# soon-yau/upgpt

Measured on AMD Instinct MI355X. Metric: 256x256 images/sec, 50-step DDIM, bs=8/GPU; UNet MFMA util %, higher is better.
Workload: dtype f16; 1 GPU; BASELINE configs[1]: bs=8/GPU, 256x256 px (latent 4x32x32), 50-step DDIM eta=0, text-only cond [B,87,768], UNet(bbox.yaml) + VAE decode, EMA weights, no CFG; batch_per_gpu=8, ddim_steps=50, batches_in_flight_per_gpu=4, lane_hw_queues=measured, parallelism=replica-dp1, one all-gather of images per batch

## Files before the change

### include/upk.h

```cpp
#ifndef UPK_H_
#define UPK_H_

#include <stddef.h>
#include <stdint.h>

#ifdef __cplusplus
extern "C" {
#endif

#define UPK_VERSION 100

#define UPK_OK 0
#define UPK_EINVAL (-1)
#define UPK_ESHAPE (-2)
#define UPK_EWORKSPACE (-3)
#define UPK_EHIP (-4)
#define UPK_ENODEV (-5)

typedef struct upk_ctx upk_ctx;
typedef void* upk_stream;

int upk_version(void);
int upk_create(upk_ctx** out, int device);
int upk_destroy(upk_ctx* ctx);
// ... 17 lines not shown
typedef struct upk_conv_desc {
  const void* x1;
  const void* x2;
  int32_t c1, c2;
  int32_t ld1, ld2;
  int32_t batch;
  int32_t in_h, in_w;
  int32_t ksize;
  int32_t stride;
  const void* w_packed;
  int32_t n_out;
  int32_t n_pad;
  const float* bias;
  const void* residual;
  int32_t ld_res;
  const float* rowvec;
  int32_t rv_batch_stride;
  int32_t rv_step_stride;
  const int32_t* step;
  void* y;
  int32_t ldy;
  void* vt;
  int32_t vt_from, vt_heads, vt_dhead, vt_ld, vt_tokens;
  int32_t flags;
  int32_t tune_cfg, tune_splitk;
  const float* ln_colsum;
  float ln_eps;
  int32_t ln_dim;
  float* gn_stats_ws;
  int32_t gn_groups;
  const void* x3;
  const void* x4;
  int32_t c3, c4;
  int32_t ld3, ld4;
  const float* gno_gamma;
  const float* gno_beta;
  void* gno_y;
  float gno_eps;
  int32_t gno_silu, gno_ld, gno_skip_y;
  float* ln_rows_out;
  const float* ln_rows_in;
  int32_t ln_rows_slots;
  const void* w_phase;
  int32_t gn_stats_cap;
  const void* pf_next;
  int64_t pf_bytes;
} upk_conv_desc;

int upk_conv2d_nhwc_f16(upk_ctx* ctx, const upk_conv_desc* d, upk_stream stream);

int upk_conv_gn_fused(upk_ctx* ctx, const upk_conv_desc* d, int* mode, int* nblk);
int upk_groupnorm_finalize_f32(upk_ctx* ctx, const float* partials, int nblk, int ld, int batch, int hw, int c,
                               int groups, float* ws, upk_stream stream);
int upk_conv_ln_rows(upk_ctx* ctx, const upk_conv_desc* d, int* slots);

typedef struct upk_mlp_desc {
  const void* x;
  int32_t ldx, m, c, inner;
  const void* w1;
  const float* b1;
  const float* u1;
  float ln_eps;
  int32_t ln_dim;
  const void* w2;
  const float* b2;
  int32_t n_out, n_pad;
  const void* residual;
  int32_t ld_res;
  void* y;
  int32_t ldy;
  float* gn_stats_ws;
  int32_t hw, rows_per_wg;
} upk_mlp_desc;
int upk_geglu_mlp_f16(upk_ctx* ctx, const upk_mlp_desc* d, upk_stream stream);
int upk_geglu_mlp_supported(upk_ctx* ctx, const upk_mlp_desc* d);

typedef struct upk_xblock_desc {
  const void* a1;
  int32_t lda, m, c, heads, d;
  const void* t0;
  int32_t ld_t0;
  const void* w_out1;
  const void* w_q;
  const void* w_out2;
  const float* vec;
  float ln_eps;
  int32_t ln_dim;
  const void* k_ctx;
  int32_t ldk, n_kv;
  const void* vt_ctx;
  int32_t vt_ld;
  float scale;
  void* y;
  int32_t ldy;
  int32_t hw, rows_per_wg;
} upk_xblock_desc;
int upk_cross_block_f16(upk_ctx* ctx, const upk_xblock_desc* d, upk_stream stream);
int upk_cross_block_supported(upk_ctx* ctx, const upk_xblock_desc* d);

typedef struct upk_hblock_desc {
  const void* x;
  int32_t ldx, m, c, heads, d;
  const void* w_in;
  const void* w_qkv;
  const float* vec;
  float ln_eps;
// ... 194 lines not shown
```

### upgpt_amd/_lib.py

```python
import contextlib
import ctypes as C
import os
import threading

import torch
from ._check import require

_HERE = os.path.dirname(os.path.abspath(__file__))
LIB_PATH = os.environ.get("UPK_LIB") or os.path.join(_HERE, "libupk.so")

SYMBOLS = [
    "upk_version", "upk_create", "upk_destroy", "upk_last_error", "upk_set_workspace", "upk_num_cus",
    "upk_pack_weight_f16", "upk_packed_weight_bytes", "upk_conv2d_nhwc_f16", "upk_gemm_f16",
    "upk_conv_autotune", "upk_conv_override", "upk_conv_num_configs", "upk_conv_config_name", "upk_conv_gn_fused",
    "upk_conv_ln_rows",
    "upk_geglu_mlp_f16", "upk_geglu_mlp_supported", "upk_cross_block_f16", "upk_cross_block_supported", "upk_head_block_f16", "upk_head_block_supported",
    "upk_attention_f16", "upk_groupnorm_nhwc_f16", "upk_groupnorm_stats_nhwc_f16", "upk_groupnorm_chunks", "upk_groupnorm_apply_nhwc_f16", "upk_groupnorm_finalize_f32", "upk_groupnorm_ws_bytes",
    "upk_layernorm_f16", "upk_timestep_embed_f16",
    "upk_nchw_f32_to_nhwc_f16", "upk_nhwc_f16_to_nchw_f32", "upk_f32_to_f16", "upk_ddim_step_f32",
    "upk_ddim_step_cfg_f32", "upk_ddim_step_edit_f32", "upk_plms_step_f32", "upk_ddpm_step_f32", "upk_attention_causal_f16", "upk_attention_qproj_f16", "upk_embed_tokens_f16",
    "upk_patchify_nchw_f32_f16", "upk_vit_assemble_f16", "upk_gather_rows_f16",
    "upk_image_finish_u8", "upk_resize_bilinear_u8", "upk_segm_boxes_u8", "upk_style_crops_u8",
    "upk_cond_bbox_u8", "upk_cond_gather_u8", "upk_cond_smpl_u8", "upk_clip_normalize_u8", "upk_ssim_ws_bytes", "upk_ssim_u8",
    "upk_lpips_input_f16", "upk_relu_pool_nhwc_f16", "upk_lpips_ws_bytes", "upk_lpips_layer_f16",
    "upk_conv2d_rect_f16", "upk_pool3_nhwc_f16", "upk_fid_input_f16", "upk_avgpool_global_f32",
    "upk_advance_step", "upk_step_autoadvance", "upk_kernel_launches", "upk_graph_begin", "upk_graph_end", "upk_graph_launch", "upk_graph_destroy",
    "upk_prof_enable", "upk_prof_collect",
    "upk_stream_create_cumask", "upk_stream_destroy", "upk_probe_placement", "upk_probe_clock",
]

F_SILU, F_GEGLU, F_OUT_F32, F_OUT_NCHW_F32, F_UPSAMPLE2X, F_PAD_ASYM = 0x1, 0x2, 0x4, 0x8, 0x10, 0x20
DDPM_X0, DDPM_CLIP = 0x1, 0x2
LAYOUT_NCHW, LAYOUT_NHWC = 0, 1
STYLE_FILL, STYLE_MASK = 0x1, 0x2
FINISH_SAMPLE, FINISH_INPUT, FINISH_DENORM = 0, 1, 2
F_QUICKGELU = 0x40
POOL_MAX, POOL_AVG = 0, 1
NUM_CLASSES = 5
CLASS_NAMES = ["igemm", "attention", "groupnorm", "layernorm", "other"]

E_NAMES = {0: "UPK_OK", -1: "UPK_EINVAL", -2: "UPK_ESHAPE", -3: "UPK_EWORKSPACE", -4: "UPK_EHIP", -5: "UPK_ENODEV"}


class UpkError(RuntimeError):
    def __init__(self, code, msg):
        super().__init__("%s: %s" % (E_NAMES.get(code, str(code)), msg))
        self.code = code


class ConvDesc(C.Structure):
    _fields_ = [
        ("x1", C.c_void_p), ("x2", C.c_void_p),
        ("c1", C.c_int32), ("c2", C.c_int32), ("ld1", C.c_int32), ("ld2", C.c_int32),
        ("batch", C.c_int32), ("in_h", C.c_int32), ("in_w", C.c_int32),
        ("ksize", C.c_int32), ("stride", C.c_int32),
        ("w_packed", C.c_void_p), ("n_out", C.c_int32), ("n_pad", C.c_int32),
        ("bias", C.c_void_p), ("residual", C.c_void_p), ("ld_res", C.c_int32),
        ("rowvec", C.c_void_p), ("rv_batch_stride", C.c_int32), ("rv_step_stride", C.c_int32),
        ("step", C.c_void_p), ("y", C.c_void_p), ("ldy", C.c_int32),
        ("vt", C.c_void_p), ("vt_from", C.c_int32), ("vt_heads", C.c_int32), ("vt_dhead", C.c_int32),
        ("vt_ld", C.c_int32), ("vt_tokens", C.c_int32), ("flags", C.c_int32),
        ("tune_cfg", C.c_int32), ("tune_splitk", C.c_int32),
        ("ln_colsum", C.c_void_p), ("ln_eps", C.c_float), ("ln_dim", C.c_int32),
        ("gn_stats_ws", C.c_void_p), ("gn_groups", C.c_int32),
        ("x3", C.c_void_p), ("x4", C.c_void_p),
        ("c3", C.c_int32), ("c4", C.c_int32), ("ld3", C.c_int32), ("ld4", C.c_int32),
        ("gno_gamma", C.c_void_p), ("gno_beta", C.c_void_p), ("gno_y", C.c_void_p), ("gno_eps", C.c_float),
        ("gno_silu", C.c_int32), ("gno_ld", C.c_int32), ("gno_skip_y", C.c_int32),
        ("ln_rows_out", C.c_void_p), ("ln_rows_in", C.c_void_p), ("ln_rows_slots", C.c_int32),
        ("w_phase", C.c_void_p), ("gn_stats_cap", C.c_int32),
# ... 42 lines not shown
    global _lib
    with _lib_lock:
        if _lib is not None and path is None:
            return _lib
        p = path or LIB_PATH
        if not os.path.exists(p):
            raise RuntimeError(
                "libupk.so not found at %s: build it with `python -m upgpt_amd.build` "
                "(hipcc --offload-arch=gfx950). There is no CPU fallback." % p)
        lib = C.CDLL(p)
        vp, i32, i64, f32 = C.c_void_p, C.c_int, C.c_longlong, C.c_float
        protos = {
            "upk_version": (C.c_int, []),
            "upk_create": (C.c_int, [C.POINTER(vp), i32]),
            "upk_destroy": (C.c_int, [vp]),
            "upk_last_error": (C.c_char_p, [vp]),
            "upk_set_workspace": (C.c_int, [vp, vp, C.c_size_t]),
            "upk_num_cus": (C.c_int, [vp]),
            "upk_pack_weight_f16": (C.c_int, [vp, vp, i32, i32, i32, i32, vp, i32, vp, i32, vp, vp]),
            "upk_packed_weight_bytes": (C.c_size_t, [i32, i32, i32, i32]),
            "upk_conv2d_nhwc_f16": (C.c_int, [vp, C.POINTER(ConvDesc), vp]),
            "upk_gemm_f16": (C.c_int, [vp, vp, i32, i32, i32, vp, i32, i32, vp, vp, i32, vp, i32, i32, vp]),
            "upk_conv_autotune": (C.c_int, [vp, C.POINTER(ConvDesc), vp, i32, C.POINTER(C.c_int), C.POINTER(C.c_int),
                                            C.POINTER(C.c_float), C.POINTER(C.c_float)]),
            "upk_conv_override": (C.c_int, [vp, i32, i32]),
            "upk_conv_num_configs": (C.c_int, []),
            "upk_conv_config_name": (C.c_char_p, [i32]),
            "upk_conv_ln_rows": (C.c_int, [vp, C.POINTER(ConvDesc), C.POINTER(C.c_int)]),
            "upk_geglu_mlp_f16": (C.c_int, [vp, C.POINTER(MlpDesc), vp]),
            "upk_geglu_mlp_supported": (C.c_int, [vp, C.POINTER(MlpDesc)]),
            "upk_cross_block_f16": (C.c_int, [vp, C.POINTER(XblockDesc), vp]),
            "upk_cross_block_supported": (C.c_int, [vp, C.POINTER(XblockDesc)]),
            "upk_head_block_f16": (C.c_int, [vp, C.POINTER(HblockDesc), vp]),
            "upk_head_block_supported": (C.c_int, [vp, C.POINTER(HblockDesc)]),
            "upk_attention_f16": (C.c_int, [vp, vp, i32, i64, vp, i32, i64, vp, i32, vp, i32, i64,
                                            i32, i32, i32, i32, i32, f32, vp]),
            "upk_attention_causal_f16": (C.c_int, [vp, vp, i32, i64, vp, i32, i64, vp, i32, vp, i32, i64,
                                                   i32, i32, i32, i32, f32, vp]),
            "upk_attention_qproj_f16": (C.c_int, [vp, vp, i32, i64, i32, i32, f32, vp, vp, vp, vp, i32, i64, vp, i32, vp,
                                                  i32, i64, i32, i32, i32, i32, i32, f32, vp]),
            "upk_embed_tokens_f16": (C.c_int, [vp, vp, vp, vp, i32, i32, i32, i32, vp, i32, vp]),
            "upk_gather_rows_f16": (C.c_int, [vp, vp, i32, vp, i32, i32, i32, vp, i32, vp]),
            "upk_patchify_nchw_f32_f16": (C.c_int, [vp, vp, i32, i32, i32, i32, i32, vp, i32, vp]),
            "upk_vit_assemble_f16": (C.c_int, [vp, vp, i32, vp, vp, i32, i32, i32, vp, i32, vp]),
            "upk_groupnorm_nhwc_f16": (C.c_int, [vp, vp, i32, i32, vp, i32, i32, i32, i32, i32, vp, vp,
                                                 f32, i32, vp, i32, vp, vp]),
            "upk_groupnorm_stats_nhwc_f16": (C.c_int, [vp, vp, i32, i32, vp, i32, i32, i32, i32, i32, vp, vp]),
            "upk_groupnorm_chunks": (C.c_int, [i32]),
            "upk_groupnorm_apply_nhwc_f16": (C.c_int, [vp, vp, i32, i32, vp, i32, i32, i32, i32, i32, vp, vp,
                                                       f32, i32, vp, i32, vp, i32, i32, i32, vp, i32, i32, vp]),
            "upk_conv_gn_fused": (C.c_int, [vp, C.POINTER(ConvDesc), C.POINTER(C.c_int), C.POINTER(C.c_int)]),
            "upk_groupnorm_finalize_f32": (C.c_int, [vp, vp, i32, i32, i32, i32, i32, i32, vp, vp]),
            "upk_groupnorm_ws_bytes": (C.c_size_t, [i32, i32]),
            "upk_layernorm_f16": (C.c_int, [vp, vp, i32, i32, i32, vp, vp, f32, vp, i32, vp]),
            "upk_timestep_embed_f16": (C.c_int, [vp, vp, i32, i32, f32, vp, i32, vp]),
            "upk_nchw_f32_to_nhwc_f16": (C.c_int, [vp, vp, i32, i32, i32, vp, i32, i32, i32, f32, vp]),
            "upk_nhwc_f16_to_nchw_f32": (C.c_int, [vp, vp, i32, i32, i32, i32, vp, vp]),
            "upk_f32_to_f16": (C.c_int, [vp, vp, i32, i32, vp, i32, vp]),
            "upk_ddim_step_f32": (C.c_int, [vp, vp, vp, vp, vp, vp, vp, vp, i32, i32, i32, i32, vp]),
            "upk_ddim_step_cfg_f32": (C.c_int, [vp, vp, vp, vp, vp, vp, vp, vp, i32, i32, i32, i32, f32, vp]),
            "upk_ddim_step_edit_f32": (C.c_int, [vp, vp, vp, vp, vp, vp, vp, i32, vp, vp, vp, vp, i32, i32, i32, i32, f32,
                                                 i32, vp]),
            "upk_plms_step_f32": (C.c_int, [vp, vp, vp, vp, vp, vp, vp, vp, i32, i32, i32, i32, f32, i32, vp]),
            "upk_ddpm_step_f32": (C.c_int, [vp, vp, vp, vp, vp, vp, vp, vp, vp, vp, vp, i32, i32, i32, i32, i32, vp]),
            "upk_image_finish_u8": (C.c_int, [vp, vp, i32, i32, i32, i32, i64, i32, i32, i32, i32, vp, i64, i32, i64, i32,
                                              C.POINTER(C.c_float), vp]),
            "upk_resize_bilinear_u8": (C.c_int, [vp, vp, i32, i32, i32, i64, i64, i32, i32, i32, i32, vp, vp, i32, vp, vp, i32,
                                                 vp, i64, i64, vp, vp, vp]),
            "upk_segm_boxes_u8": (C.c_int, [vp, vp, i64, i64, vp, i64, i64, i32, i32, i32, C.POINTER(C.c_uint32), i32, vp, vp]),
            "upk_style_crops_u8": (C.c_int, [vp, vp, i64, i64, vp, i64, i64, i32, i32, i32, C.POINTER(C.c_uint32), i32, vp,
                                             C.POINTER(C.c_int32), C.POINTER(C.c_int32), i32, C.POINTER(C.c_float), vp, vp, vp,
                                             vp, vp]),
            "upk_cond_bbox_u8": (C.c_int, [vp, vp, i64, i64, i32, i32, i32, vp, vp, i32, i32, vp, vp, vp]),
            "upk_cond_gather_u8": (C.c_int, [vp, vp, i64, i64, i32, i32, i32, vp, vp, i32, i32, C.POINTER(C.c_float), vp, vp]),
            "upk_cond_smpl_u8": (C.c_int, [vp, vp, i64, i64, i32, i32, i32, vp, vp]),
            "upk_clip_normalize_u8": (C.c_int, [vp, vp, i64, i64, vp, i32, i32, i32, C.POINTER(C.c_float), vp, vp]),
            "upk_ssim_ws_bytes": (C.c_size_t, [i32, i32, i32, i32]),
            "upk_ssim_u8": (C.c_int, [vp, vp, i64, i64, vp, i64, i64, i32, i32, i32, i32, vp, vp, C.c_size_t, vp]),
            "upk_lpips_input_f16": (C.c_int, [vp, vp, i32, i64, i64, i32, i32, i32, i32, C.POINTER(C.c_float), vp, i64, vp]),
            "upk_relu_pool_nhwc_f16": (C.c_int, [vp, vp, i32, i32, i32, i32, i32, vp, i32, vp]),
            "upk_lpips_ws_bytes": (C.c_size_t, [i32, i32, i32]),
            "upk_lpips_layer_f16": (C.c_int, [vp, vp, vp, i32, i64, i32, i32, i32, vp, i32, vp, vp, C.c_size_t, vp]),
            "upk_conv2d_rect_f16": (C.c_int, [vp, vp, i32, i32, i32, i32, i32, i32, i32, i32, i32, i32, vp, i32, i32, vp, i32, vp,
                                              i32, vp]),
            "upk_pool3_nhwc_f16": (C.c_int, [vp, vp, i32, i32, i32, i32, i32, i32, i32, vp, i32, vp]),
            "upk_fid_input_f16": (C.c_int, [vp, vp, i32, i64, i64, i32, i32, i32, i32, i32, i32, vp, i64, vp]),
            "upk_avgpool_global_f32": (C.c_int, [vp, vp, i32, i32, i32, i32, vp, vp]),
            "upk_advance_step": (C.c_int, [vp, vp, vp]),
            "upk_step_autoadvance": (C.c_int, [vp, vp]),
            "upk_kernel_launches": (C.c_longlong, [vp, i32]),
            "upk_graph_begin": (C.c_int, [vp, vp]),
            "upk_graph_end": (C.c_int, [vp, vp, C.POINTER(vp)]),
            "upk_graph_launch": (C.c_int, [vp, vp, vp]),
            "upk_graph_destroy": (C.c_int, [vp, vp]),
            "upk_prof_enable": (C.c_int, [vp, i32]),
            "upk_prof_collect": (C.c_int, [vp, C.POINTER(C.c_double), C.POINTER(C.c_longlong)]),
            "upk_stream_create_cumask": (C.c_int, [vp, C.POINTER(C.c_uint32), i32, C.POINTER(vp)]),
            "upk_stream_destroy": (C.c_int, [vp, vp]),
            "upk_probe_placement": (C.c_int, [vp, vp, i32, i32, vp]),
            "upk_probe_clock": (C.c_int, [vp, vp, i64, vp]),
        }
        require(sorted(protos) == sorted(SYMBOLS), "ctypes prototypes and SYMBOLS differ", RuntimeError)
        for name, (res, args) in protos.items():
            fn = getattr(lib, name)
            fn.restype = res
            fn.argtypes = args
# ... 371 lines not shown
```

### upgpt_amd/build.py

```python
import hashlib
import os
import shutil
import subprocess
import sys
from concurrent.futures import ThreadPoolExecutor

HERE = os.path.dirname(os.path.abspath(__file__))
CSRC = os.path.join(HERE, "csrc")
OUT = os.environ.get("UPK_LIB") or os.path.join(HERE, "libupk.so")
SOURCES = ["igemm.hip", "bigtile.hip", "astat.hip", "mlp.hip", "xblock.hip", "attention.hip", "norm.hip", "misc.hip", "image.hip",
           "metrics.hip", "lpips.hip", "inception.hip", "resize.hip", "styles.hip", "batch.hip"]
FILE_FLAGS = {"attention.hip": ["-mllvm", "-amdgpu-mfma-vgpr-form", "-fno-honor-nans", "-mno-amdgpu-ieee"],
              "image.hip": ["-ffp-contract=off"], "lpips.hip": ["-ffp-contract=off"],
              "inception.hip": ["-ffp-contract=off"], "resize.hip": ["-ffp-contract=off"],
              "styles.hip": ["-ffp-contract=off"], "batch.hip": ["-ffp-contract=off"]}
ARCH = "gfx950"


def _hipcc():
    for cand in (os.environ.get("HIPCC"), shutil.which("hipcc"), "/opt/rocm/bin/hipcc"):
        if cand and os.path.exists(cand):
            return cand
    raise RuntimeError("hipcc not found: libupk.so cannot be built")


def _source_hash():
    h = hashlib.sha256()
    files = sorted(os.path.join(CSRC, f) for f in os.listdir(CSRC)) + [os.path.join(HERE, "..", "include", "upk.h")]
    for path in files:
        h.update(os.path.basename(path).encode())
        with open(path, "rb") as f:
            h.update(f.read())
    h.update((ARCH + " " + os.environ.get("UPK_CXXFLAGS", "") + repr(sorted(FILE_FLAGS.items()))).encode())
    return h.hexdigest()


def _stale():
    if os.environ.get("UPK_FORCE_BUILD", "0") == "1" or not os.path.exists(OUT):
        return True
    try:
        with open(OUT + ".sha256") as f:
            return f.read().strip() != _source_hash()
    except OSError:
        return True


def build(force=False, verbose=True):
    if not force and not _stale():
        return OUT
    hipcc = _hipcc()
    objdir = os.path.join(HERE, "build" + ("_dev" if os.environ.get("UPK_LIB") else ""))
    os.makedirs(objdir, exist_ok=True)
    flags = ["--offload-arch=" + ARCH, "-O3", "-std=c++17", "-fPIC", "-ffp-contract=fast",
             "-Wno-unused-result", "-I", os.path.join(HERE, "..", "include")]
    flags += os.environ.get("UPK_CXXFLAGS", "").split()

    headers = sorted(os.path.join(CSRC, f) for f in os.listdir(CSRC) if f.endswith(".h")) + [
        os.path.join(HERE, "..", "include", "upk.h")]

    def obj_hash(src):
        h = hashlib.sha256()
        for path in [os.path.join(CSRC, src)] + headers:
            with open(path, "rb") as f:
                h.update(f.read())
# ... 39 lines not shown
```

### upgpt_amd/engine.py

```python
import ctypes as C
import os

import torch

from . import _lib as L
from . import knobs as K
from ._check import require
from .arch import UNetArch, VAEArch
from .emitter import Act, Emitter, Program
from .packing import (PW, PackedUNet, PackedVAEDecoder, PackedVAEEncoder, PackedVGG16, Packer, _rup,
                      geglu_rows_map, head_pad, pad_rows_map, qproj_pack, vgg16_convs)
from .tuning import TUNE_CACHE, TuneCache


class UNetPlan(Emitter):

    def __init__(self, ctx, packed: PackedUNet, B, H, W, n_ctx, rows, mode):
        super().__init__(ctx)
        require(mode in ("forward", "sampler"), "UNetPlan mode must be 'forward' or 'sampler'", ValueError)
        self.pk, self.arch = packed, packed.arch
        self.B, self.H, self.W, self.n_ctx, self.rows, self.mode = B, H, W, n_ctx, rows, mode
        a = self.arch
        mc, te = a.model_channels, a.time_embed_dim
        self.cin_pad = _rup(a.in_channels, 32)
# ... 157 lines not shown
            self.taps["output_blocks.%d" % i] = x
        self.conv(P, x, self.pk.w["out.2"], nchw_out=self.eps, gn=(*self.pk.v["out.0"], 1e-5, True, self.gn_ws))

    def close(self):
        for attr in ("_sampler_state", "_sampler_state_cfg", "_plms_state", "_plms_state_cfg", "_ddpm_state"):
            st = self.__dict__.pop(attr, None)
            if st is not None:
                st.close()

    def load_sampler_inputs(self, x, c_concat, c_cross, in_channels, rows_key, t_rows):
        C = x.shape[1]
        self.load_x_nchw(x, 0, 0)
        ncat = 0
        if c_concat is not None:
            ncat = c_concat.shape[1]
            self.load_x_nchw(c_concat, C, self.cin_pad)
        require(C + ncat == in_channels, lambda: "latent %d + concat %d != UNet in_channels %d" % (C, ncat, in_channels),
                ValueError)
        self.load_context(c_cross)
        if getattr(self, "_t_rows_key", None) != rows_key:
            self.t_rows.copy_(torch.as_tensor(t_rows))
            self._t_rows_key = rows_key

    def load_context(self, context):
        require(tuple(context.shape) == (self.B, self.n_ctx, self.arch.context_dim), lambda: "context shape %s != plan %s" % (tuple(context.shape), (self.B, self.n_ctx, self.arch.context_dim)), ValueError)
        self.ctx32.copy_(context.reshape(self.B * self.n_ctx, -1).to(self.dev, torch.float32), non_blocking=True)

    def load_x_nchw(self, x, c_off=0, zero_pad_to=0):
        x = x.to(self.dev, torch.float32).contiguous()
        require(x.shape[0] == self.B and tuple(x.shape[2:]) == (self.H, self.W), lambda: "stem input %s does not match the plan (B=%d, %dx%d)" % (tuple(x.shape), self.B, self.H, self.W), ValueError)
        self.ctx.nchw_to_nhwc(x, self.B, x.shape[1], self.H * self.W, self.xin.t, self.xin.ld, c_off, zero_pad_to, 1.0)


class VAEDecodePlan(Emitter):

    def __init__(self, ctx, packed: PackedVAEDecoder, B, h, w, scale_factor):
        super().__init__(ctx)
        self.pk, self.arch = packed, packed.arch
        a = self.arch
        self.B, self.h, self.w = B, h, w
        f = a.factor
        self.z = self.alloc(B, a.embed_dim, h, w, dtype=torch.float32)
        self.img = self.alloc(B, a.out_ch, h * f, w * f, dtype=torch.float32)
        self.gn_ws = self.alloc(max(64, ctx.groupnorm_ws_bytes(B, h * f * w * f) // 4), dtype=torch.float32)
        self.prog = Program(ctx)
        P, W_, V_ = self.prog, packed.w, packed.v
        zin = Act(self.alloc(B * h * w, _rup(a.embed_dim, 32), zero=True), B, h, w, a.embed_dim)
        lib, hh, chk, z = self.lib, self.hctx, self._chk, self.z
        inv = 1.0 / float(scale_factor)
        P.add(lambda s: chk(lib.upk_nchw_f32_to_nhwc_f16(hh, z.data_ptr(), B, a.embed_dim, h * w, zin.t.data_ptr(),
                                                         zin.ld, 0, 0, inv, s)))
        x = self.conv(P, zin, W_["post_quant_conv"],
                      out=Act(self.alloc(B * h * w, _rup(a.z_channels, 32), zero=True), B, h, w, a.z_channels))
        for Lr in a.decoder:
            n = Lr.name
            if Lr.kind == "conv":
                x = self.conv(P, x, W_[n], gn_stats=K.vae_gn_byproduct(x.M))
            elif Lr.kind == "resnet":
                h1 = self.conv(P, x, W_[n + ".conv1"], gn=(*V_[n + ".norm1"], 1e-6, True, self.gn_ws), gn_stats=K.vae_gn_byproduct(x.M))
                sk = self.conv(P, x, W_[n + ".nin_shortcut"]) if Lr.cin != Lr.cout else x
                x = self.conv(P, h1, W_[n + ".conv2"], residual=sk, gn=(*V_[n + ".norm2"], 1e-6, True, self.gn_ws),
                              gn_stats=K.vae_gn_byproduct(x.M))
            elif Lr.kind == "attn":
                c, HW = Lr.ch, x.H * x.W
                xn = self.groupnorm(P, x, *V_[n + ".norm"], 1e-6, False, self.gn_ws)
                qk = Act(self.alloc(x.M, 2 * c), x.B, x.H, x.W, 2 * c)
                vt_ld = _rup(HW, 32)
                vt = self.alloc(x.B, 1, c, vt_ld, zero=True)
                self.conv(P, xn, W_[n + ".qkv"], out=qk,
                          vt=dict(t=vt, heads=1, dhead=c, ld=vt_ld, tokens=HW, **{"from": 2 * c}))
                ao = Act(self.alloc(x.M, c), x.B, x.H, x.W, c)
                self.attention(P, qk.t, 2 * c, HW * 2 * c, qk.t[:, c:], 2 * c, HW * 2 * c, vt, vt_ld, ao.t, c, HW * c,
                               x.B, 1, HW, HW, c, int(c) ** -0.5)
                x = self.conv(P, ao, W_[n + ".proj_out"], residual=x, gn_stats=K.vae_gn_byproduct(x.M))
            elif Lr.kind == "upconv":
                x = self.conv(P, x, W_[n], flags=L.F_UPSAMPLE2X)
            elif Lr.kind == "norm_out":
                x = self.groupnorm(P, x, *V_[n], 1e-6, True, self.gn_ws)
            elif Lr.kind == "conv_out":
                self.conv(P, x, W_[n], nchw_out=self.img)
        self.graph = None

    def run(self, z):
        z = z.to(self.dev, torch.float32).contiguous()
        require(tuple(z.shape) == tuple(self.z.shape), lambda: repr((z.shape, self.z.shape)), ValueError)
        self.z.copy_(z)
        self.prog.run()
        return self.img


class VAEEncodePlan(Emitter):

    def __init__(self, ctx, packed: PackedVAEEncoder, B, H, W):
        super().__init__(ctx)
        self.pk, self.arch = packed, packed.arch
        a = self.arch
        f = a.factor
        require(H % f == 0 and W % f == 0, lambda: "image size must be a multiple of %d" % f, ValueError)
        self.x = self.alloc(B, a.in_channels, H, W, dtype=torch.float32)
        self.moments = self.alloc(B, 2 * a.embed_dim, H // f, W // f, dtype=torch.float32)
        self.gn_ws = self.alloc(max(64, ctx.groupnorm_ws_bytes(B, H * W) // 4), dtype=torch.float32)
        self.prog = Program(ctx)
        P, W_, V_ = self.prog, packed.w, packed.v
        xin = Act(self.alloc(B * H * W, _rup(a.in_channels, 32), zero=True), B, H, W, a.in_channels)
        lib, hh, chk, xs = self.lib, self.hctx, self._chk, self.x
        P.add(lambda s: chk(lib.upk_nchw_f32_to_nhwc_f16(hh, xs.data_ptr(), B, a.in_channels, H * W,
                                                         xin.t.data_ptr(), xin.ld, 0, 0, 1.0, s)))
        x = xin
        for Lr in a.encoder:
            n = Lr.name
            if Lr.kind == "conv":
                x = self.conv(P, x, W_[n], gn_stats=K.vae_gn_byproduct(x.M))
            elif Lr.kind == "resnet":
                h1 = self.conv(P, x, W_[n + ".conv1"], gn=(*V_[n + ".norm1"], 1e-6, True, self.gn_ws), gn_stats=K.vae_gn_byproduct(x.M))
                sk = self.conv(P, x, W_[n + ".nin_shortcut"]) if Lr.cin != Lr.cout else x
                x = self.conv(P, h1, W_[n + ".conv2"], residual=sk, gn=(*V_[n + ".norm2"], 1e-6, True, self.gn_ws),
                              gn_stats=K.vae_gn_byproduct(x.M))
            elif Lr.kind == "attn":
                c, HW = Lr.ch, x.H * x.W
                xn = self.groupnorm(P, x, *V_[n + ".norm"], 1e-6, False, self.gn_ws)
                qk = Act(self.alloc(x.M, 2 * c), x.B, x.H, x.W, 2 * c)
                vt_ld = _rup(HW, 32)
                vt = self.alloc(x.B, 1, c, vt_ld, zero=True)
                self.conv(P, xn, W_[n + ".qkv"], out=qk,
                          vt=dict(t=vt, heads=1, dhead=c, ld=vt_ld, tokens=HW, **{"from": 2 * c}))
                ao = Act(self.alloc(x.M, c), x.B, x.H, x.W, c)
                self.attention(P, qk.t, 2 * c, HW * 2 * c, qk.t[:, c:], 2 * c, HW * 2 * c, vt, vt_ld, ao.t, c, HW * c,
                               x.B, 1, HW, HW, c, int(c) ** -0.5)
                x = self.conv(P, ao, W_[n + ".proj_out"], residual=x)
            elif Lr.kind == "downconv":
                x = self.conv(P, x, W_[n], stride=2, flags=L.F_PAD_ASYM)
            elif Lr.kind == "norm_out":
                x = self.groupnorm(P, x, *V_[n], 1e-6, True, self.gn_ws)
            elif Lr.kind == "conv_out":
# ... 354 lines not shown
```

### upgpt_amd/knobs.py

```python
import os

VAE_GN_BYPRODUCT = os.environ.get("UPGPT_VAE_GN_BYPRODUCT", "0")
VAE_GN_MINM = int(os.environ.get("UPGPT_VAE_GN_MINM", "131072"))


def vae_gn_byproduct(M):
    return VAE_GN_BYPRODUCT == "1" or (VAE_GN_BYPRODUCT == "auto" and M >= VAE_GN_MINM)
UPS_PHASES = os.environ.get("UPGPT_UPS_PHASES", "1") == "1"
LN_ROWS = os.environ.get("UPGPT_LN_ROWS", "1") == "1"
QPROJ_FUSE = os.environ.get("UPGPT_QPROJ_FUSE", "1") == "1"
GN_REDUCE_APPLY = os.environ.get("UPGPT_GN_REDUCE_APPLY", "1") == "1"
MLP_FUSE = os.environ.get("UPGPT_MLP_FUSE", "auto")
MLP_ROWS = int(os.environ.get("UPGPT_MLP_ROWS", "0"))
XBLOCK = os.environ.get("UPGPT_XBLOCK", "auto")
XB_ROWS = int(os.environ.get("UPGPT_XB_ROWS", "0"))
HB_ROWS = int(os.environ.get("UPGPT_HB_ROWS", "0"))
HBLOCK = os.environ.get("UPGPT_HBLOCK", "auto")
HBLOCK_GN = os.environ.get("UPGPT_HBLOCK_GN", "1") == "1"
WEIGHT_PREFETCH = os.environ.get("UPGPT_WEIGHT_PREFETCH", "auto")
WEIGHT_PREFETCH_AHEAD = int(os.environ.get("UPGPT_WEIGHT_PREFETCH_AHEAD", "1"))
WEIGHT_PREFETCH_MAX = int(os.environ.get("UPGPT_WEIGHT_PREFETCH_MAX", str(32 << 20)))
LN_LAUNCH_US = 5.0
```

### upgpt_amd/packing.py

```python
import torch

from . import knobs as K
from ._check import require
from .arch import UNetArch, VAEArch


def _rup(v, m):
    return (v + m - 1) // m * m



def head_pad(d):
    for p in (32, 64, 128, 256, 512):
        if d <= p:
            return p
    raise NotImplementedError("attention head dim %d > 512" % d)


class PW:
    __slots__ = ("w", "n_pad", "bias", "n_out", "k_packed", "ksize", "n_real", "k_real", "ln_colsum", "k_append", "w_phase")


class SharedPacks:

# ... 79 lines not shown
        p.k_append = 0
        p.w_phase = None
        b = None
        if bias:
            bs = [self.get(n + ".bias") for n in names]
            b = (bs[0] if len(bs) == 1 else torch.cat(bs, 0)).float()
        if ln_bias is not None:
            b = ln_bias if b is None else b + ln_bias
            p.ln_colsum = rows_packed(w.half().float().sum(dim=1))
        if b is not None:
            p.bias = rows_packed(b)
        return p

    def add_upsample_phases(self, p, name):
        w = self.get(name + ".weight").float().to(self.dev)
        require(w.dim() == 4 and w.shape[-1] == 3 and w.shape[-2] == 3, "upsample phase weights need a 3x3 conv weight", ValueError)
        taps = {(0, 0): (0,), (0, 1): (1, 2), (1, 0): (0, 1), (1, 1): (2,)}
        parts = []
        for py in (0, 1):
            for px in (0, 1):
                wp = torch.zeros(w.shape[0], w.shape[1], 2, 2, device=self.dev)
                for ty in (0, 1):
                    for tx in (0, 1):
                        for ky in taps[(py, ty)]:
                            for kx in taps[(px, tx)]:
                                wp[:, :, ty, tx] += w[:, :, ky, kx]
                packed, n_pad = self.ctx.pack_weight(wp.contiguous())
                require(n_pad == p.n_pad, "phase weight rows differ from the 3x3 weight's", RuntimeError)
                parts.append(packed.reshape(-1))
        p.w_phase = torch.cat(parts).contiguous()
        return p

    def append_1x1(self, main, skip):
        require(skip.ksize == 1 and skip.n_pad == main.n_pad and skip.n_out == main.n_out and main.ln_colsum is None, "append_1x1: the appended weight must be a 1x1 with the main weight's rows", ValueError)
        p = PW()
        p.w = torch.cat([main.w.reshape(-1), skip.w.reshape(-1)])
        p.n_pad, p.n_out, p.ksize, p.k_packed, p.n_real = main.n_pad, main.n_out, main.ksize, main.k_packed, main.n_real
        p.k_append = skip.k_packed
        p.k_real = main.k_real + skip.k_real
        p.ln_colsum = None
        bs = [b for b in (main.bias, skip.bias) if b is not None]
        p.bias = None if not bs else (bs[0] if len(bs) == 1 else bs[0] + bs[1])
        return p

    def pack_product(self, outer, inner):
        wo = self.get(outer + ".weight").float()
        wo = wo.reshape(wo.shape[0], -1)
        wi = self.get(inner + ".weight").float()
        prod = {"p.weight": (wo @ wi).contiguous(), "p.bias": wo @ self.get(inner + ".bias").float()}
        return Packer(self.ctx, lambda n: prod[n]).pack("p")

    def vec(self, name):
        return self.get(name).float().contiguous()


def qproj_pack(w, gamma, beta, heads, dh, dp, cq, dev):
    C_ = w.shape[1]
    wf = torch.zeros(heads, dp, cq, dtype=torch.float32, device=dev)
    wf[:, :dh, :C_] = (w.float().to(dev) * gamma.float().to(dev)[None, :]).reshape(heads, dh, C_)
    bias = torch.zeros(heads, dp, dtype=torch.float32, device=dev)
    bias[:, :dh] = (w.float().to(dev) @ beta.float().to(dev)).reshape(heads, dh)
    w16 = wf.half()
    colsum = w16.float().sum(dim=2)
    r = torch.arange(dp, device=dev)
    kd, t, m = r // 32, (r % 32) // 16, r % 16
    src = 32 * kd + 8 * (m // 4) + 4 * t + (m % 4)
    return w16[:, src, :].contiguous(), colsum.reshape(-1).contiguous(), bias.reshape(-1).contiguous()


def pad_rows_map(parts, heads, dh, dp):
    j = torch.arange(parts * heads * dp)
    part, r = j // (heads * dp), j % (heads * dp)
    h, d = r // dp, r % dp
    return torch.where(d < dh, part * heads * dh + h * dh + d, torch.full_like(j, -1))


def geglu_rows_map(inner):
    j = torch.arange(2 * inner)
    blk, r = j // 64, j % 64
    return torch.where(r < 32, blk * 32 + r, inner + blk * 32 + (r - 32))


class PackedUNet:

    def __init__(self, ctx, arch: UNetArch, get):
        pk = Packer(ctx, get)
        self.arch = arch
        mc, te = arch.model_channels, arch.time_embed_dim
        if mc % 32:
            raise NotImplementedError("model_channels must be a multiple of 32 (got %d)" % mc)
        w = {}
        w["time_embed.0"] = pk.pack("time_embed.0")
        w["time_embed.2"] = pk.pack("time_embed.2")
        v = {}

        def norm(name):
            v[name] = (pk.vec(name + ".weight"), pk.vec(name + ".bias"))

        for Lr in arch.all_layers():
            n = Lr.name
            if Lr.kind == "conv":
                w[n] = pk.pack(n, cin_packed=_rup(Lr.cin, 32))
            elif Lr.kind == "res":
                norm(n + ".in_layers.0")
                w[n + ".in_layers.2"] = pk.pack(n + ".in_layers.2")
                w[n + ".emb_layers.1"] = pk.pack(n + ".emb_layers.1")
# ... 5 lines not shown
            elif Lr.kind == "st":
                if Lr.depth != 1:
                    raise NotImplementedError("transformer_depth != 1")
                heads, dh = Lr.heads, Lr.dhead
                dp = head_pad(dh)
                hd = heads * dp
                norm(n + ".norm")
                w[n + ".proj_in"] = pk.pack(n + ".proj_in")
                t = n + ".transformer_blocks.0"
                to_out_cols = pad_rows_map(1, heads, dh, dp)
                for sfx, fold in (("", None), ("_ln", True)):
                    w[t + ".attn1.qkv" + sfx] = pk.pack(
                        [t + ".attn1.to_q", t + ".attn1.to_k", t + ".attn1.to_v"], row_map=pad_rows_map(3, heads, dh, dp),
                        bias=False, n_out=2 * hd, ln=(t + ".norm1") if fold else None)
                    w[t + ".attn2.q" + sfx] = pk.pack(t + ".attn2.to_q", row_map=pad_rows_map(1, heads, dh, dp),
                                                      bias=False, ln=(t + ".norm2") if fold else None)
                    w[t + ".ff.geglu" + sfx] = pk.pack(t + ".ff.net.0.proj", row_map=geglu_rows_map(4 * heads * dh),
                                                       n_out=4 * heads * dh, ln=(t + ".norm3") if fold else None)
                if dp in (32, 64) and Lr.ch % 224 == 0:
                    w[t + ".attn2.qproj"] = qproj_pack(get(t + ".attn2.to_q.weight"), get(t + ".norm2.weight"),
                                                       get(t + ".norm2.bias"), heads, dh, dp, Lr.ch, ctx.device)
                w[t + ".attn1.to_out"] = pk.pack(t + ".attn1.to_out.0", col_map=to_out_cols)
                w[t + ".attn2.kv"] = pk.pack([t + ".attn2.to_k", t + ".attn2.to_v"],
                                             row_map=pad_rows_map(2, heads, dh, dp), bias=False, n_out=hd)
                w[t + ".attn2.to_out"] = pk.pack(t + ".attn2.to_out.0", col_map=to_out_cols)
                pi, qkv = w[n + ".proj_in"], w[t + ".attn1.qkv_ln"]
                if pi.n_pad == Lr.ch and qkv.n_pad == 3 * hd and pi.ksize == 1:
                    vec = torch.cat([pi.bias, qkv.ln_colsum, qkv.bias])
                    w[t + ".hblock.vec"] = torch.cat([vec, vec.new_zeros(-vec.numel() % 256)]).contiguous()
                o1, o2, ql = w[t + ".attn1.to_out"], w[t + ".attn2.to_out"], w[t + ".attn2.q_ln"]
                if o1.n_pad == Lr.ch and o2.n_pad == Lr.ch and ql.n_pad == hd:
                    vec = torch.cat([o1.bias, ql.ln_colsum, ql.bias, o2.bias])
                    w[t + ".xblock.vec"] = torch.cat([vec, vec.new_zeros(-vec.numel() % 256)]).contiguous()
                inner = heads * dh
                w[t + ".ff.out"] = pk.pack(t + ".ff.net.2")
                for k in ("norm1", "norm2", "norm3"):
                    norm(t + "." + k)
                w[n + ".proj_out"] = pk.pack(n + ".proj_out")
                w[n + ".ff.out+proj_out"] = pk.append_1x1(pk.pack_product(n + ".proj_out", t + ".ff.net.2"),
                                                          w[n + ".proj_out"])
            elif Lr.kind == "down":
                w[n + ".op"] = pk.pack(n + ".op")
            elif Lr.kind == "up":
                w[n + ".conv"] = pk.add_upsample_phases(pk.pack(n + ".conv"), n + ".conv")
        norm("out.0")
        w["out.2"] = pk.pack("out.2")
        self.w, self.v = w, v


class PackedVAEDecoder:
    def __init__(self, ctx, arch: VAEArch, get):
        pk = Packer(ctx, get)
        self.arch = arch
        w, v = {}, {}

        def norm(name):
            v[name] = (pk.vec("decoder." + name + ".weight"), pk.vec("decoder." + name + ".bias"))

        w["post_quant_conv"] = pk.pack("post_quant_conv", cin_packed=_rup(arch.embed_dim, 32))
        for Lr in arch.decoder:
            n, d = Lr.name, "decoder." + Lr.name
            if Lr.kind in ("conv", "conv_out"):
                w[n] = pk.pack(d, cin_packed=_rup(Lr.cin, 32))
            elif Lr.kind == "resnet":
                norm(n + ".norm1")
                w[n + ".conv1"] = pk.pack(d + ".conv1")
                norm(n + ".norm2")
                w[n + ".conv2"] = pk.pack(d + ".conv2")
                if Lr.cin != Lr.cout:
                    w[n + ".nin_shortcut"] = pk.pack(d + ".nin_shortcut")
            elif Lr.kind == "attn":
                if Lr.ch not in (32, 64, 128, 256, 512):
                    raise NotImplementedError("VAE AttnBlock width %d" % Lr.ch)
                norm(n + ".norm")
                w[n + ".qkv"] = pk.pack([d + ".q", d + ".k", d + ".v"], n_out=2 * Lr.ch)
                w[n + ".proj_out"] = pk.pack(d + ".proj_out")
            elif Lr.kind == "upconv":
                w[n] = pk.add_upsample_phases(pk.pack(d), d)
            elif Lr.kind == "norm_out":
                norm(n)
        self.w, self.v = w, v


class PackedVAEEncoder:
    def __init__(self, ctx, arch: VAEArch, get):
        pk = Packer(ctx, get)
        self.arch = arch
        w, v = {}, {}

        def norm(name):
            v[name] = (pk.vec("encoder." + name + ".weight"), pk.vec("encoder." + name + ".bias"))

        for Lr in arch.encoder:
            n, d = Lr.name, "encoder." + Lr.name
            if Lr.kind in ("conv", "conv_out"):
                w[n] = pk.pack(d, cin_packed=_rup(Lr.cin, 32))
            elif Lr.kind == "resnet":
                norm(n + ".norm1")
                w[n + ".conv1"] = pk.pack(d + ".conv1")
                norm(n + ".norm2")
                w[n + ".conv2"] = pk.pack(d + ".conv2")
                if Lr.cin != Lr.cout:
                    w[n + ".nin_shortcut"] = pk.pack(d + ".nin_shortcut")
            elif Lr.kind == "attn":
                if Lr.ch not in (32, 64, 128, 256, 512):
                    raise NotImplementedError("VAE AttnBlock width %d" % Lr.ch)
                norm(n + ".norm")
                w[n + ".qkv"] = pk.pack([d + ".q", d + ".k", d + ".v"], n_out=2 * Lr.ch)
                w[n + ".proj_out"] = pk.pack(d + ".proj_out")
            elif Lr.kind == "downconv":
                w[n] = pk.pack(d)
            elif Lr.kind == "norm_out":
                norm(n)
        zc2 = arch.encoder[-1].cout
        w["quant_conv"] = pk.pack("quant_conv", cin_packed=_rup(zc2, 32))
        self.w, self.v = w, v
# ... 124 lines not shown
```

Before: 97.88 images/s.

## Fuse VAE final GroupNorm+SiLU with 3-channel conv_out into one kernel

Adds a dedicated HIP kernel that applies the decoder's final GroupNorm and SiLU on the fly while loading a halo tile into LDS. It then computes the 3x3 conv to 3 output channels in fp32 FMA and writes NCHW f32 directly. This removes the normalized activation write/read round-trip and avoids running a padded MFMA implicit GEMM with only 3 real output channels. It reuses GN stats from fused producers when available, otherwise it launches a stats kernel. The trade-off is scalar FMA compute instead of MFMA, plus extra fp32 weight packing.

```diff
diff --git a/include/upk.h b/include/upk.h
--- a/include/upk.h
+++ b/include/upk.h
@@ -93,6 +93,10 @@
 int upk_conv_gn_fused(upk_ctx* ctx, const upk_conv_desc* d, int* mode, int* nblk);
 int upk_groupnorm_finalize_f32(upk_ctx* ctx, const float* partials, int nblk, int ld, int batch, int hw, int c,
                                int groups, float* ws, upk_stream stream);
+int upk_vae_tail_supported(upk_ctx* ctx, int batch, int h, int w, int c, int ldx, int groups, int n_out);
+int upk_vae_tail_f16(upk_ctx* ctx, const void* x, int ldx, int batch, int h, int w, int c, int groups,
+                     const float* gamma, const float* beta, float eps, const float* stats_ws, const float* w_taps,
+                     const float* bias, float* y_nchw, upk_stream stream);
 int upk_conv_ln_rows(upk_ctx* ctx, const upk_conv_desc* d, int* slots);
 
 typedef struct upk_mlp_desc {
diff --git a/upgpt_amd/_lib.py b/upgpt_amd/_lib.py
--- a/upgpt_amd/_lib.py
+++ b/upgpt_amd/_lib.py
@@ -16,6 +16,7 @@
     "upk_conv_ln_rows",
     "upk_geglu_mlp_f16", "upk_geglu_mlp_supported", "upk_cross_block_f16", "upk_cross_block_supported", "upk_head_block_f16", "upk_head_block_supported",
     "upk_attention_f16", "upk_groupnorm_nhwc_f16", "upk_groupnorm_stats_nhwc_f16", "upk_groupnorm_chunks", "upk_groupnorm_apply_nhwc_f16", "upk_groupnorm_finalize_f32", "upk_groupnorm_ws_bytes",
+    "upk_vae_tail_supported", "upk_vae_tail_f16",
     "upk_layernorm_f16", "upk_timestep_embed_f16",
     "upk_nchw_f32_to_nhwc_f16", "upk_nhwc_f16_to_nchw_f32", "upk_f32_to_f16", "upk_ddim_step_f32",
     "upk_ddim_step_cfg_f32", "upk_ddim_step_edit_f32", "upk_plms_step_f32", "upk_ddpm_step_f32", "upk_attention_causal_f16", "upk_attention_qproj_f16", "upk_embed_tokens_f16",
@@ -164,6 +165,8 @@
             "upk_conv_gn_fused": (C.c_int, [vp, C.POINTER(ConvDesc), C.POINTER(C.c_int), C.POINTER(C.c_int)]),
             "upk_groupnorm_finalize_f32": (C.c_int, [vp, vp, i32, i32, i32, i32, i32, i32, vp, vp]),
             "upk_groupnorm_ws_bytes": (C.c_size_t, [i32, i32]),
+            "upk_vae_tail_supported": (C.c_int, [vp, i32, i32, i32, i32, i32, i32, i32]),
+            "upk_vae_tail_f16": (C.c_int, [vp, vp, i32, i32, i32, i32, i32, i32, vp, vp, f32, vp, vp, vp, vp, vp]),
             "upk_layernorm_f16": (C.c_int, [vp, vp, i32, i32, i32, vp, vp, f32, vp, i32, vp]),
             "upk_timestep_embed_f16": (C.c_int, [vp, vp, i32, i32, f32, vp, i32, vp]),
             "upk_nchw_f32_to_nhwc_f16": (C.c_int, [vp, vp, i32, i32, i32, vp, i32, i32, i32, f32, vp]),
diff --git a/upgpt_amd/build.py b/upgpt_amd/build.py
--- a/upgpt_amd/build.py
+++ b/upgpt_amd/build.py
@@ -9,7 +9,7 @@
 CSRC = os.path.join(HERE, "csrc")
 OUT = os.environ.get("UPK_LIB") or os.path.join(HERE, "libupk.so")
 SOURCES = ["igemm.hip", "bigtile.hip", "astat.hip", "mlp.hip", "xblock.hip", "attention.hip", "norm.hip", "misc.hip", "image.hip",
-           "metrics.hip", "lpips.hip", "inception.hip", "resize.hip", "styles.hip", "batch.hip"]
+           "metrics.hip", "lpips.hip", "inception.hip", "resize.hip", "styles.hip", "batch.hip", "vae_tail.hip"]
 FILE_FLAGS = {"attention.hip": ["-mllvm", "-amdgpu-mfma-vgpr-form", "-fno-honor-nans", "-mno-amdgpu-ieee"],
               "image.hip": ["-ffp-contract=off"], "lpips.hip": ["-ffp-contract=off"],
               "inception.hip": ["-ffp-contract=off"], "resize.hip": ["-ffp-contract=off"],
diff --git a/upgpt_amd/csrc/vae_tail.hip b/upgpt_amd/csrc/vae_tail.hip
--- /dev/null
+++ b/upgpt_amd/csrc/vae_tail.hip
@@ -0,0 +1,198 @@
+#include "common.h"
+
+namespace {
+
+constexpr int VT_TW = 32, VT_TH = 8;
+constexpr int VT_HW = VT_TW + 2, VT_HH = VT_TH + 2;
+constexpr int VT_NPIX = VT_HW * VT_HH;
+constexpr int VT_CK = 16;
+constexpr int VT_PSTR = VT_CK + 4;
+constexpr int VT_NVEC = VT_NPIX * (VT_CK / 8);
+constexpr int VT_NLD = (VT_NVEC + 255) / 256;
+constexpr int VT_VPP = VT_CK / 8;
+constexpr int VT_CMAX = 256;
+
+struct VaeTailArgs {
+  const f16* x;
+  int ldx;
+  int h, w, c;
+  int groups, cpg, nchunks;
+  const float* gamma;
+  const float* beta;
+  float eps;
+  const float* stats;
+  const float* bias;
+  float* y;
+  int tiles_x;
+};
+
+__global__ __launch_bounds__(256) void vae_tail_kernel(const VaeTailArgs a, const float* __restrict__ wt) {
+  __shared__ __attribute__((aligned(16))) float tile[VT_NPIX * VT_PSTR];
+  __shared__ __attribute__((aligned(16))) float scale[VT_CMAX], shift[VT_CMAX];
+  __shared__ float smean[UPK_GN_GROUPS_MAX], srstd[UPK_GN_GROUPS_MAX];
+  double* part = (double*)tile;
+  int t, b;
+  upk_xcd_xb(t, b);
+  const int tid = threadIdx.x;
+  const int ty = t / a.tiles_x, tx = t - ty * a.tiles_x;
+  const int y0 = ty * VT_TH, x0 = tx * VT_TW;
+
+  {
+    const int q = tid >> 2, sub = tid & 3;
+    if (q < a.groups * 2) {
+      const float* ws = a.stats + (long)b * a.nchunks * a.groups * 2 + q;
+      float v[UPK_GN_MAX_CHUNKS / 4];
+#pragma unroll
+      for (int k = 0; k < UPK_GN_MAX_CHUNKS / 4; ++k) {
+        const int idx = sub + 4 * k;
+        v[k] = ws[(long)(idx < a.nchunks ? idx : 0) * a.groups * 2];
+      }
+      double acc = 0.0;
+#pragma unroll
+      for (int k = 0; k < UPK_GN_MAX_CHUNKS / 4; ++k) acc += (double)(sub + 4 * k < a.nchunks ? v[k] : 0.f);
+      part[tid] = acc;
+    }
+    __syncthreads();
+    if (tid < a.groups) {
+      const double s = ((part[tid * 8 + 0] + part[tid * 8 + 1]) + part[tid * 8 + 2]) + part[tid * 8 + 3];
+      const double ss = ((part[tid * 8 + 4] + part[tid * 8 + 5]) + part[tid * 8 + 6]) + part[tid * 8 + 7];
+      const double n = (double)a.h * a.w * a.cpg;
+      const double mean = s / n;
+      double var = ss / n - mean * mean;
+      if (var < 0.0) var = 0.0;
+      smean[tid] = (float)mean;
+      srstd[tid] = (float)(1.0 / sqrt(var + (double)a.eps));
+    }
+    __syncthreads();
+    for (int ch = tid; ch < a.c; ch += 256) {
+      const int g = ch / a.cpg;
+      const float sc = srstd[g] * a.gamma[ch];
+      scale[ch] = sc;
+      shift[ch] = a.beta[ch] - smean[g] * sc;
+    }
+  }
+
+  int lds_off[VT_NLD];
+  long src_off[VT_NLD];
+  bool inside[VT_NLD];
+#pragma unroll
+  for (int k = 0; k < VT_NLD; ++k) {
+    const int i = tid + k * 256;
+    const int ic = i < VT_NVEC ? i : 0;
+    const int hp = ic / VT_VPP, v = ic % VT_VPP;
+    const int hy = hp / VT_HW, hx = hp - hy * VT_HW;
+    const int gy = y0 + hy - 1, gx = x0 + hx - 1;
+    inside[k] = i < VT_NVEC && gy >= 0 && gy < a.h && gx >= 0 && gx < a.w;
+    const int cy = min(max(gy, 0), a.h - 1), cx = min(max(gx, 0), a.w - 1);
+    src_off[k] = (((long)b * a.h + cy) * a.w + cx) * a.ldx + v * 8;
+    lds_off[k] = i < VT_NVEC ? hp * VT_PSTR + v * 8 : -1;
+  }
+
+  const int py = tid >> 5, px = tid & 31;
+  f32x2 acc[3];
+#pragma unroll
+  for (int o = 0; o < 3; ++o) acc[o] = f32x2{0.f, 0.f};
+
+  const int nck = a.c / VT_CK;
+  for (int ck = 0; ck < nck; ++ck) {
+    f16x8 xv[VT_NLD];
+#pragma unroll
+    for (int k = 0; k < VT_NLD; ++k) xv[k] = *(const f16x8*)(a.x + src_off[k] + ck * VT_CK);
+    __syncthreads();
+    const int ch = ck * VT_CK + (tid % VT_VPP) * 8;
+    const f32x4 sc0 = *(const f32x4*)(scale + ch), sc1 = *(const f32x4*)(scale + ch + 4);
+    const f32x4 sh0 = *(const f32x4*)(shift + ch), sh1 = *(const f32x4*)(shift + ch + 4);
+    constexpr float NL2E = -1.44269504088896340736f;
+    const f32x4 nc0 = sc0 * NL2E, nc1 = sc1 * NL2E, nh0 = sh0 * NL2E, nh1 = sh1 * NL2E;
+#pragma unroll
+    for (int k = 0; k < VT_NLD; ++k) {
+      if (lds_off[k] < 0) continue;
+      f32x4 o0, o1;
+#pragma unroll
+      for (int j = 0; j < 4; ++j) {
+        const float x0 = (float)xv[k][j], x1 = (float)xv[k][j + 4];
+        const float v0 = x0 * sc0[j] + sh0[j], v1 = x1 * sc1[j] + sh1[j];
+        const float e0 = __builtin_amdgcn_exp2f(x0 * nc0[j] + nh0[j]), e1 = __builtin_amdgcn_exp2f(x1 * nc1[j] + nh1[j]);
+        o0[j] = inside[k] ? v0 * __builtin_amdgcn_rcpf(1.0f + e0) : 0.f;
+        o1[j] = inside[k] ? v1 * __builtin_amdgcn_rcpf(1.0f + e1) : 0.f;
+      }
+      *(f32x4*)(tile + lds_off[k]) = o0;
+      *(f32x4*)(tile + lds_off[k] + 4) = o1;
+    }
+    __syncthreads();
+    const f32x2* wc = (const f32x2*)wt + (long)ck * 9 * (VT_CK / 2) * 3;
+#pragma unroll
+    for (int ky = 0; ky < 3; ++ky)
+#pragma unroll
+      for (int kx = 0; kx < 3; ++kx) {
+        const float* src = tile + ((py + ky) * VT_HW + px + kx) * VT_PSTR;
+        const f32x2* wtap = wc + (ky * 3 + kx) * (VT_CK / 2) * 3;
+#pragma unroll
+        for (int q = 0; q < VT_CK / 4; ++q) {
+          const f32x4 v = *(const f32x4*)(src + q * 4);
+          const f32x2 lo = {v[0], v[1]}, hi = {v[2], v[3]};
+#pragma unroll
+          for (int o = 0; o < 3; ++o) {
+            acc[o] = __builtin_elementwise_fma(lo, wtap[(q * 2) * 3 + o], acc[o]);
+            acc[o] = __builtin_elementwise_fma(hi, wtap[(q * 2 + 1) * 3 + o], acc[o]);
+          }
+        }
+      }
+  }
+  const int gy = y0 + py, gx = x0 + px;
+  if (gy < a.h && gx < a.w) {
+#pragma unroll
+    for (int o = 0; o < 3; ++o)
+      a.y[(((long)b * 3 + o) * a.h + gy) * a.w + gx] = (acc[o][0] + acc[o][1]) + a.bias[o];
+  }
+}
+
+bool vae_tail_domain(int batch, int h, int w, int c, int ldx, int groups, int n_out) {
+  if (batch <= 0 || h <= 0 || w <= 0 || n_out != 3) return false;
+  if (c <= 0 || c % 32 || c > VT_CMAX || ldx < c || (ldx & 7)) return false;
+  if (groups <= 0 || groups > UPK_GN_GROUPS_MAX || c % groups) return false;
+  if (batch > 65535) return false;
+  return true;
+}
+
+}
+
+extern "C" int upk_vae_tail_supported(upk_ctx* ctx, int batch, int h, int w, int c, int ldx, int groups, int n_out) {
+  (void)ctx;
+  return vae_tail_domain(batch, h, w, c, ldx, groups, n_out) ? 1 : 0;
+}
+
+extern "C" int upk_vae_tail_f16(upk_ctx* ctx, const void* x, int ldx, int batch, int h, int w, int c, int groups,
+                                const float* gamma, const float* beta, float eps, const float* stats_ws,
+                                const float* w_taps, const float* bias, float* y_nchw, upk_stream stream_) {
+  if (!ctx) return UPK_EINVAL;
+  if (!x || !gamma || !beta || !stats_ws || !w_taps || !bias || !y_nchw)
+    return upk_fail(ctx, UPK_EINVAL, "vae_tail: null pointer");
+  if (((uintptr_t)x & 15) || ((uintptr_t)w_taps & 15))
+    return upk_fail(ctx, UPK_EINVAL, "vae_tail: x and w_taps must be 16-byte aligned");
+  if (!vae_tail_domain(batch, h, w, c, ldx, groups, 3))
+    return upk_fail(ctx, UPK_ESHAPE, "vae_tail: B=%d %dx%d C=%d ld=%d groups=%d outside the kernel's domain", batch, h, w,
+                    c, ldx, groups);
+  VaeTailArgs a;
+  a.x = (const f16*)x;
+  a.ldx = ldx;
+  a.h = h;
+  a.w = w;
+  a.c = c;
+  a.groups = groups;
+  a.cpg = c / groups;
+  int ppc;
+  upk_gn_chunking(h * w, &a.nchunks, &ppc);
+  a.gamma = gamma;
+  a.beta = beta;
+  a.eps = eps;
+  a.stats = stats_ws;
+  a.bias = bias;
+  a.y = y_nchw;
+  a.tiles_x = (w + VT_TW - 1) / VT_TW;
+  const int tiles = a.tiles_x * ((h + VT_TH - 1) / VT_TH);
+  hipStream_t stream = (hipStream_t)stream_;
+  upk_prof_scope prof(ctx, UPK_CLS_OTHER, stream);
+  hipLaunchKernelGGL(vae_tail_kernel, dim3(tiles, batch), dim3(256), 0, stream, a, w_taps);
+  return upk_check_launch(ctx, "vae_tail");
+}
diff --git a/upgpt_amd/engine.py b/upgpt_amd/engine.py
--- a/upgpt_amd/engine.py
+++ b/upgpt_amd/engine.py
@@ -233,6 +233,7 @@
                                                          zin.ld, 0, 0, inv, s)))
         x = self.conv(P, zin, W_["post_quant_conv"],
                       out=Act(self.alloc(B * h * w, _rup(a.z_channels, 32), zero=True), B, h, w, a.z_channels))
+        tail_norm = None
         for Lr in a.decoder:
             n = Lr.name
             if Lr.kind == "conv":
@@ -257,10 +258,56 @@
             elif Lr.kind == "upconv":
                 x = self.conv(P, x, W_[n], flags=L.F_UPSAMPLE2X)
             elif Lr.kind == "norm_out":
-                x = self.groupnorm(P, x, *V_[n], 1e-6, True, self.gn_ws)
+                if self.tail_ok(x, packed.tail):
+                    tail_norm = V_[n]
+                else:
+                    x = self.groupnorm(P, x, *V_[n], 1e-6, True, self.gn_ws)
             elif Lr.kind == "conv_out":
-                self.conv(P, x, W_[n], nchw_out=self.img)
+                if tail_norm is not None:
+                    self.vae_tail(P, x, *tail_norm, 1e-6, self.gn_ws, packed.tail, self.img)
+                else:
+                    self.conv(P, x, W_[n], nchw_out=self.img)
         self.graph = None
+
+    def tail_ok(self, x, tail):
+        if K.VAE_TAIL == "0" or tail is None:
+            return False
+        return bool(self.lib.upk_vae_tail_supported(self.hctx, x.B, x.H, x.W, x.C, x.ld, 32, int(tail[1].numel())))
+
+    def vae_tail(self, P, x, gamma, beta, eps, ws, tail, img):
+        wt, bias = tail
+        lib, h, chk = self.lib, self.hctx, self._chk
+        hw = x.H * x.W
+        a = (x.t.data_ptr(), x.ld, x.B, x.H, x.W, x.C, 32, gamma.data_ptr(), beta.data_ptr(), float(eps))
+        b = (wt.data_ptr(), bias.data_ptr(), img.data_ptr())
+        armed = self._arm_gn_sources([x])
+
+        def run(s):
+            stats = ws.data_ptr()
+            mode = 0
+            if armed is not None:
+                src, sws = armed[0]
+                if isinstance(src, Emitter.GnProvider):
+                    mode, nb, ld = 2, src.nblk, src.ld
+                else:
+                    m_, n_ = C.c_int(0), C.c_int(0)
+                    chk(lib.upk_conv_gn_fused(h, C.byref(src), C.byref(m_), C.byref(n_)))
+                    mode, nb, ld = m_.value, n_.value, src.n_pad
+                if mode == 2:
+                    chk(lib.upk_groupnorm_finalize_f32(h, sws.data_ptr(), nb, ld, x.B, hw, x.C, 32, stats, s))
+                elif mode == 1:
+                    stats = sws.data_ptr()
+                else:
+                    mode = 0
+            if mode == 0:
+                chk(lib.upk_groupnorm_stats_nhwc_f16(h, x.t.data_ptr(), x.C, x.ld, None, 0, 0, x.B, hw, 32, stats, s))
+            chk(lib.upk_vae_tail_f16(h, *a, stats, *b, s))
+
+        P.add(run, x, gamma, beta, ws, wt, bias, img, armed, cls="other", label="vae_tail M%d C%d" % (x.M, x.C))
+        P.n_launch += 1
+        fl = 2 * x.M * 9 * x.C * 3
+        P.igemm_flops += fl
+        P.flops[-1] = fl
 
     def run(self, z):
         z = z.to(self.dev, torch.float32).contiguous()
diff --git a/upgpt_amd/knobs.py b/upgpt_amd/knobs.py
--- a/upgpt_amd/knobs.py
+++ b/upgpt_amd/knobs.py
@@ -6,6 +6,9 @@
 
 def vae_gn_byproduct(M):
     return VAE_GN_BYPRODUCT == "1" or (VAE_GN_BYPRODUCT == "auto" and M >= VAE_GN_MINM)
+
+
+VAE_TAIL = os.environ.get("UPGPT_VAE_TAIL", "auto")
 UPS_PHASES = os.environ.get("UPGPT_UPS_PHASES", "1") == "1"
 LN_ROWS = os.environ.get("UPGPT_LN_ROWS", "1") == "1"
 QPROJ_FUSE = os.environ.get("UPGPT_QPROJ_FUSE", "1") == "1"
diff --git a/upgpt_amd/packing.py b/upgpt_amd/packing.py
--- a/upgpt_amd/packing.py
+++ b/upgpt_amd/packing.py
@@ -155,6 +155,18 @@
 
     def vec(self, name):
         return self.get(name).float().contiguous()
+
+    def tail3(self, name):
+        w = self.get(name + ".weight").float()
+        if w.dim() != 4 or tuple(w.shape[2:]) != (3, 3) or w.shape[0] != 3 or w.shape[1] % 32:
+            return None
+        return tail3_layout(w.to(self.dev)), self.get(name + ".bias").float().to(self.dev).contiguous()
+
+
+def tail3_layout(w):
+    cin = w.shape[1]
+    t = w.half().float().permute(1, 2, 3, 0).reshape(cin // 16, 8, 2, 9, 3)
+    return t.permute(0, 3, 1, 4, 2).contiguous()
 
 
 def qproj_pack(w, gamma, beta, heads, dh, dp, cq, dev):
@@ -266,6 +278,7 @@
     def __init__(self, ctx, arch: VAEArch, get):
         pk = Packer(ctx, get)
         self.arch = arch
+        self.tail = None
         w, v = {}, {}
 
         def norm(name):
@@ -276,6 +289,8 @@
             n, d = Lr.name, "decoder." + Lr.name
             if Lr.kind in ("conv", "conv_out"):
                 w[n] = pk.pack(d, cin_packed=_rup(Lr.cin, 32))
+                if Lr.kind == "conv_out":
+                    self.tail = pk.tail3(d)
             elif Lr.kind == "resnet":
                 norm(n + ".norm1")
                 w[n + ".conv1"] = pk.pack(d + ".conv1")
```

Result: no change. 97.75 images/s, median of 2 (-0.1%).
